# cdglissov/recurrent-flows-msc

Measured on AMD Instinct MI355X. Metric: frames/sec, RFN SM-MNIST 64x64 train step (fwd+bwd+Adam), higher is better.
Workload: dtype f32 (forward convolutions fp32-grade: fused scaled-fp16 split f16x3s / three-piece bf16x6 split; gradient convolutions bf16x3 split MFMA; fp32 accumulate everywhere); 1 GPU; RFN SM-MNIST 64x64 canonical (K=10 L=5 Hd=256 h=200 z=56), global_batch=32, seq_len=20, train step; global_batch=32, seq_len=20, parallelism=dp1

## Files before the change

include/rfn_hip.h:

```cpp
#ifndef RFN_HIP_H
#define RFN_HIP_H

#ifdef __cplusplus
extern "C" {
#endif

typedef void* rfn_stream_t;

int rfn_abi_version(void);
const char* rfn_last_error(void);

int rfn_squeeze2d_f32(const float* x, long x_ns, float* y, long y_ns, int N, int C, int H, int W, int undo,
                      rfn_stream_t stream);

int rfn_channel_stats_f32(const float* x, long x_ns, float* mean, float* var_unbiased, int N, int C, int HW,
                          rfn_stream_t stream);

int rfn_actnorm_invconv_fwd_f32(const float* x, long x_ns, const float* bias, const float* logs, const float* Wm,
                                float* z, long z_ns, int N, int C, int HW, rfn_stream_t stream);
int rfn_actnorm_invconv_bwd_f32(const float* x, long x_ns, const float* bias, const float* logs, const float* Wm,
                                const float* gz, long gz_ns, float* gx, long gx_ns, float* gW, float* gbias,
                                float* glogs, int N, int C, int HW, rfn_stream_t stream);
#define RFN_INVCONV_MAX_STEPS 32
#define RFN_INVCONV_MAX_CHANNELS 96
// ... 50 lines not shown
typedef struct {
    const float* w1;
    const float* w2;
    const float* w3;
    float* dst;
    int Cin, C;
} rfn_po_pack_desc;
int rfn_coupling_po_supported(int N, int C, int Cc, int Hd, int H, int W);
long rfn_coupling_po_packed_bytes(int Cin, int C);
int rfn_coupling_po_pack(const void* descs_device, int n, rfn_stream_t stream);
int rfn_coupling_po_fwd(const float* z, long z_ns, const float* cond, long cond_ns, const void* wpk, const float* n1b,
                        const float* n1l, const float* n2b, const float* n2l, float* h1, long h1_ns, float* h2,
                        long h2_ns, float* P, long P_ns, float* m1, float* m2, int N, int C, int Cc, int H, int W, int act,
                        rfn_stream_t stream);
long rfn_coupling_po_mask_floats(int N, int H, int W);
int rfn_coupling_po_bwd_supported(int N, int C, int H, int W);
long rfn_coupling_po_bwd_packed_bytes(int C);
int rfn_coupling_po_pack_bwd(const void* descs_device, int n, rfn_stream_t stream);
long rfn_coupling_po_bwd_part_floats(int N, int H, int W);
int rfn_coupling_po_bwd(const float* go, long go_ns, const void* wpk, const float* n1l, const float* n2l,
                        const float* m_h1, const float* m_h2, float* ga2, long ga2_ns, float* ga1, long ga1_ns,
                        float* part, int N, int C, int H, int W, int act, rfn_stream_t stream);
int rfn_coupling_po_bwd_finish(const float* const* part, const float* const* w1, const float* const* gw1,
                               const float* const* n1b, const float* const* w2, const float* const* gw2,
                               const float* const* n2b, float* const* out, int n, int nblk, int K1,
                               rfn_stream_t stream);

int rfn_gather_affine_f32(const float* P, const float* o_in, long o_ns, const float* b3, const float* l3, float* o_out,
                          float* z, long z_ns, const float* scale, const float* scale_shift, float* logdet,
                          int clamp_type, int N, int C, int H, int W, rfn_stream_t stream);
// ... 265 lines not shown
```

recurrent-flows-msc_amd/csrc/coupling_po.hip:

```cpp
#include "conv_common.h"

typedef _Float16 f16x8 __attribute__((ext_vector_type(8)));

#define PO_HD 256
#define PO_TAP_PAIRS 5
#define PO_WAVES 4
#define PO_ROUND_PX (32 * PO_WAVES)

struct POGeom {
    int NG, NP, NS1;
    int quad_frags;
    int c3;
    int total_frags;
};
__host__ __device__ static inline POGeom po_geom(int Cin, int C, bool bwd = false) {
    POGeom g;
    g.NG = (Cin + 7) / 8;
    g.NP = bwd ? 0 : (9 * C + 31) / 32;
    g.NS1 = PO_TAP_PAIRS * g.NG;
    g.quad_frags = g.NG * 40 + 4 * 32;
    g.c3 = 1 + 2 * g.quad_frags;
    g.total_frags = g.c3 + 4 * 8 * g.NP;
    return g;
}

__host__ __device__ constexpr int po_gs1(int NG) { return NG > 5 ? 3 : 5; }
__host__ __device__ constexpr int po_gs3(int NP) { return NP > 3 ? 2 : 4; }
__host__ __device__ constexpr int po_group_base(int NG, int NP, int idx) {
    const int QF = NG * 40 + 128, GS1 = po_gs1(NG), NG1 = 5 * NG / GS1, F1 = 8 * GS1;
    return idx < NG1 ? 1 + idx * F1
         : idx < NG1 + 4 ? 1 + NG * 40 + (idx - NG1) * 32
         : idx < 2 * NG1 + 4 ? 1 + QF + (idx - NG1 - 4) * F1
         : idx < 2 * NG1 + 8 ? 1 + QF + NG * 40 + (idx - 2 * NG1 - 4) * 32
         : 1 + 2 * QF + (idx - 2 * NG1 - 8) * 2 * NP * po_gs3(NP);
}
__host__ __device__ constexpr int po_image_positions(int W) {
    return W * W >= PO_ROUND_PX ? (PO_ROUND_PX / W + 2) * (W + 2) : (PO_ROUND_PX / (W * W)) * (W + 2) * (W + 2);
}
__host__ __device__ constexpr int po_slot_frags(int NG, int NP) {
    const int f1 = 8 * po_gs1(NG), f3 = 2 * NP * po_gs3(NP);
    return (f1 > 32 ? f1 : 32) > f3 ? (f1 > 32 ? f1 : 32) : f3;
}
__host__ __device__ constexpr int po_group_size(int NG, int NP, int idx) {
    const int GS1 = po_gs1(NG), NG1 = 5 * NG / GS1, F1 = 8 * GS1;
    return idx < NG1 ? F1 : idx < NG1 + 4 ? 32 : idx < 2 * NG1 + 4 ? F1 : idx < 2 * NG1 + 8 ? 32 : 2 * NP * po_gs3(NP);
}

using POPackDesc = rfn_po_pack_desc;
static_assert(sizeof(rfn_po_pack_desc) == 40, "rfn_po_pack_desc layout is part of the ABI");

__host__ __device__ static inline void po_scale_for_max(float m, float* sc, float* inv) {
    unsigned bits;
    memcpy(&bits, &m, 4);
    int E = (int)((bits >> 23) & 0xff);
    if (E < 40) E = 40;
    if (E > 250) E = 250;
    const unsigned sb = (unsigned)(268 - E) << 23, ib = (unsigned)(E - 14) << 23;
    memcpy(sc, &sb, 4);
    memcpy(inv, &ib, 4);
}
// ... 40 lines not shown
#pragma unroll
    for (int c = 0; c < 3; ++c) scw[c] = 1.0f / d.dst[c];
    const int n1 = 8 * g.NS1, n2 = 8 * 16, n3 = g.NP * 16;
    const long n_items = (long)(n1 + n2 + n3) * 64;
    for (long it = (long)blockIdx.x * blockDim.x + threadIdx.x; it < n_items; it += (long)gridDim.x * blockDim.x) {
        const int lane = (int)(it & 63);
        int k = (int)(it >> 6);
        const int r = lane & 31, kk = lane >> 5;
        float v[8];
#pragma unroll
        for (int j = 0; j < 8; ++j) v[j] = 0.f;
        long frag0;
        float sc;
        if (k < n1) {
            const int a = k / g.NS1, s = k % g.NS1;
            frag0 = 1 + (long)(a >> 2) * g.quad_frags + (s / 5) * 40 + ((s % 5) * 4 + (a & 3)) * 2;
            sc = scw[0];
            const int tp = s / g.NG, gg = s % g.NG, tap = 2 * tp + kk;
            if (tap < 9) {
#pragma unroll
                for (int j = 0; j < 8; ++j) {
                    const int ci = 8 * gg + j;
                    if (ci < Cin)
                        v[j] = BWD ? d.w3[((long)ci * PO_HD + (32 * a + r)) * 9 + (8 - tap)]
                                   : d.w1[((long)(32 * a + r) * Cin + ci) * 9 + tap];
                }
            }
        } else if (k < n1 + n2) {
            k -= n1;
            const int a2 = k >> 4, s = k & 15;
            frag0 = 1 + (long)(s >> 3) * g.quad_frags + g.NG * 40 + ((s & 7) >> 1) * 32 + ((s & 1) * 8 + a2) * 2;
            sc = scw[1];
#pragma unroll
            for (int j = 0; j < 8; ++j) {
                const int c1 = 16 * s + 8 * (j >> 2) + 4 * kk + (j & 3);
                v[j] = BWD ? d.w2[(long)c1 * PO_HD + (32 * a2 + r)] : d.w2[(long)(32 * a2 + r) * PO_HD + c1];
            }
        } else {
            k -= n1 + n2;
            const int jt = k >> 4, s = k & 15;
            frag0 = g.c3 + (long)(s >> 2) * (8 * g.NP) + ((s & 3) * g.NP + jt) * 2;
            sc = scw[2];
            const int R = 32 * jt + r;
            if (R < 9 * d.C) {
                const int tap = R / d.C, co = R % d.C;
#pragma unroll
                for (int j = 0; j < 8; ++j) {
                    const int c2 = 16 * s + 8 * (j >> 2) + 4 * kk + (j & 3);
                    v[j] = d.w3[((long)co * PO_HD + c2) * 9 + tap];
                }
            }
        }
        f16x8 hi, lo;
        po_split_f16(v, sc, hi, lo);
        dst[frag0 * 64 + lane] = hi;
        dst[(frag0 + 1) * 64 + lane] = lo;
    }
}

extern "C" long rfn_coupling_po_packed_bytes(int Cin, int C) { return (long)po_geom(Cin, C).total_frags * 1024; }
extern "C" long rfn_coupling_po_bwd_packed_bytes(int C) { return (long)po_geom(C, C, true).total_frags * 1024; }

extern "C" int rfn_coupling_po_pack(const void* descs_device, int n, rfn_stream_t stream) {
    RFN_CHECK_ARG(descs_device && n >= 0, -1);
    if (n == 0) return 0;
    hipLaunchKernelGGL(po_pack_scale_kernel<false>, dim3(3, n), dim3(256), 0, (hipStream_t)stream,
                       reinterpret_cast<const POPackDesc*>(descs_device));
    hipLaunchKernelGGL(po_pack_fwd_kernel<false>, dim3(16, n), dim3(256), 0, (hipStream_t)stream,
                       reinterpret_cast<const POPackDesc*>(descs_device));
    RFN_LAUNCH_CHECK();
    return 0;
}

extern "C" int rfn_coupling_po_pack_bwd(const void* descs_device, int n, rfn_stream_t stream) {
    RFN_CHECK_ARG(descs_device && n >= 0, -1);
    if (n == 0) return 0;
// ... 68 lines not shown
        float s01 = (bit0 ? t4[1] : t4[0]) +
                    __int_as_float(__builtin_amdgcn_update_dpp(0, __float_as_int(bit0 ? t4[0] : t4[1]), 0xB1, 0xF, 0xF, true));
        float s23 = (bit0 ? t4[3] : t4[2]) +
                    __int_as_float(__builtin_amdgcn_update_dpp(0, __float_as_int(bit0 ? t4[2] : t4[3]), 0xB1, 0xF, 0xF, true));
        psum[q] += (bit1 ? s23 : s01) +
                   __int_as_float(__builtin_amdgcn_update_dpp(0, __float_as_int(bit1 ? s01 : s23), 0x4E, 0xF, 0xF, true));
    }
}

__device__ __forceinline__ int po_exp_of(const float m) {
    int E = (int)((__float_as_uint(m) >> 23) & 0xff);
    E = E < 40 ? 40 : E;
    return E > 250 ? 250 : E;
}

template <int NG, int NP, int LOGW, int ACT, bool BWD>
__global__ __launch_bounds__(64 * PO_WAVES) void coupling_po_fwd_kernel(const POFwdParams p) {
    constexpr int W = 1 << LOGW, HW = W * W, IW = W + 2;
    constexpr int FPR = HW >= PO_ROUND_PX ? 1 : PO_ROUND_PX / HW;
    constexpr int RROWS = HW >= PO_ROUND_PX ? PO_ROUND_PX / W : W;
    constexpr int FPOS = (RROWS + 2) * IW, IPOS = FPR * FPOS;
    constexpr int PO_ITEMS = (NG * IPOS + 64 * PO_WAVES - 1) / (64 * PO_WAVES);
    constexpr int RPF_SHIFT = HW >= PO_ROUND_PX ? 2 * LOGW - 7 : 0;
    constexpr int GS1 = po_gs1(NG), NG1 = 5 * NG / GS1;
    constexpr int GS3 = po_gs3(NP), NG3 = 16 / GS3;
    constexpr bool RT = NG > 5;
    constexpr bool LATE = RT || (BWD && NG > 1);
    constexpr bool NOHOIST = LATE || NG == 5;
    static_assert((5 * NG) % GS1 == 0 && (!RT || NG % GS1 == 0), "conv1 grouping");
    constexpr int G3 = 2 * NP * GS3;
    constexpr int Y1 = 2 * GS1, Y3 = G3 / 4;
    static_assert(G3 % 4 == 0, "a group's fragments are shared evenly by the four waves");
    constexpr int SLOTF = po_slot_frags(NG, NP);
    constexpr int SLOT = SLOTF * 1024;
    extern __shared__ __attribute__((aligned(16))) unsigned char lds[];
    constexpr int NGRP = 2 * NG1 + 8 + (BWD ? 0 : NG3);
    float* par = reinterpret_cast<float*>(lds + 3 * SLOT);
    float* red = par + 1024;
    f16x8* img = reinterpret_cast<f16x8*>(lds + 3 * SLOT + 4096 + 64);
    float* gsum = reinterpret_cast<float*>(lds + 3 * SLOT + 4096 + 64 + 2 * NG * IPOS * 16);
    const int tid = threadIdx.x, lane = tid & 63;
    const int wave = __builtin_amdgcn_readfirstlane(tid >> 6);
    const int l31 = lane & 31, kk = lane >> 5;
    const int Cin = p.Ch + p.Cc;
    constexpr unsigned ch_bytes = (unsigned)HW * 4u;

    for (int c = tid; c < 256; c += 64 * PO_WAVES) {
        par[c] = BWD ? 0.f : p.n1b[c];
        par[256 + c] = expf(p.n1l[c]);
        par[512 + c] = BWD ? 0.f : p.n2b[c];
        par[768 + c] = expf(p.n2l[c]);
    }
    float ps1[BWD ? 8 : 1][4], ps2[BWD ? 8 : 1][4];
#pragma unroll
    for (int a = 0; a < (BWD ? 8 : 1); ++a)
#pragma unroll
        for (int q = 0; q < 4; ++q) ps1[a][q] = ps2[a][q] = 0.f;
    const bool lbit0 = lane & 1, lbit1 = lane & 2;
    const float* hdr = reinterpret_cast<const float*>(p.wpk);
// ... 3 lines not shown
    int sl = 2;
    auto dma = [&](const int base, const int nfr, const int slot) {
        const unsigned char* src = p.wpk + (long)(base + wave) * 1024 + lane * 16;
        unsigned char* dst = lds + slot * SLOT + wave * 1024;
        for (int i = wave; i < nfr; i += PO_WAVES, src += PO_WAVES * 1024, dst += PO_WAVES * 1024)
            __builtin_amdgcn_global_load_lds((const __attribute__((address_space(1))) void*)src,
                                             (__attribute__((address_space(3))) void*)dst, 16, 0, 0);
    };
#define PO_BOUNDARY(IDX, YOUNGER)                                                                          \
    do {                                                                                                   \
        po_wait_vm<(YOUNGER) < 63 ? (YOUNGER) : 63>();                                                     \
        __builtin_amdgcn_s_barrier();                                                                      \
        const int free_slot = sl;                                                                          \
        sl = sl == 2 ? 0 : sl + 1;                                                                         \
        const int n2_ = (IDX) + 2;                                                                         \
        if (n2_ < NGRP) dma(po_group_base(NG, NP, n2_), po_group_size(NG, NP, n2_), free_slot);            \
        else if (more) dma(po_group_base(NG, NP, n2_ - NGRP), po_group_size(NG, NP, n2_ - NGRP), free_slot); \
    } while (0)

    const auto rs_h1 = __builtin_amdgcn_make_buffer_rsrc(p.h1, 0, 0xFFFFFFFFu, 0x00020000);
    const auto rs_h2 = __builtin_amdgcn_make_buffer_rsrc(p.h2, 0, 0xFFFFFFFFu, 0x00020000);

    float raw[PO_ITEMS][8];
    auto stage_load = [&](const int rnd) {
        const int n0_ = FPR > 1 ? rnd * FPR : rnd >> RPF_SHIFT;
        const int y0_ = FPR > 1 ? 0 : ((rnd & ((1 << RPF_SHIFT) - 1)) * PO_ROUND_PX) >> LOGW;
        int tid_ = tid;
        if (NOHOIST) asm volatile("" : "+v"(tid_));
#pragma unroll
        for (int it = 0; it < PO_ITEMS; ++it) {
            const int item = tid_ + it * 64 * PO_WAVES;
            const bool live = item < NG * IPOS;
            const int g = live ? item / IPOS : 0, pos = live ? item - g * IPOS : 0;
            const int fr = FPR > 1 ? pos / FPOS : 0, rem = pos - fr * FPOS;
            const int iy = rem / IW, ix = rem - iy * IW;
            const int gy = y0_ - 1 + iy, gx = ix - 1;
            const bool ok = live && gy >= 0 && gy < W && gx >= 0 && gx < W;
            const int off = ok ? gy * W + gx : 0;
            const float* zb = p.z + (long)(n0_ + fr) * p.z_ns;
            const float* cb = p.cond + (long)(n0_ + fr) * p.cond_ns;
#pragma unroll
            for (int j = 0; j < 8; ++j) {
                const int ci = 8 * g + j;
                const int cc = ci < Cin ? ci : 0;
                const float* src = cc < p.Ch ? zb + (long)cc * HW : cb + (long)(cc - p.Ch) * HW;
                raw[it][j] = src[off];
            }
        }
    };
    float u1_next = 0.f;
    auto stage_finish = [&](const int rnd) {
        const int y0_ = FPR > 1 ? 0 : ((rnd & ((1 << RPF_SHIFT) - 1)) * PO_ROUND_PX) >> LOGW;
        float vm = 0.f;
        int tid_ = tid;
        if (NOHOIST) asm volatile("" : "+v"(tid_));
#pragma unroll
        for (int it = 0; it < PO_ITEMS; ++it) {
            const int item = tid_ + it * 64 * PO_WAVES;
            const bool live = item < NG * IPOS;
            const int g = live ? item / IPOS : 0, pos = live ? item - g * IPOS : 0;
            const int rem = FPR > 1 ? pos % FPOS : pos;
            const int iy = rem / IW, ix = rem - iy * IW;
            const int gy = y0_ - 1 + iy, gx = ix - 1;
            const bool ok = live && gy >= 0 && gy < W && gx >= 0 && gx < W;
#pragma unroll
            for (int j = 0; j < 8; ++j) {
                raw[it][j] = (ok && 8 * g + j < Cin) ? raw[it][j] : 0.f;
                vm = fmaxf(vm, fabsf(raw[it][j]));
            }
        }
#pragma unroll
        for (int off = 32; off > 0; off >>= 1) vm = fmaxf(vm, __shfl_xor(vm, off, 64));
        if (lane == 0) red[wave] = vm;
        asm volatile("s_waitcnt lgkmcnt(0)" ::: "memory");
        __builtin_amdgcn_s_barrier();
        vm = fmaxf(fmaxf(red[0], red[1]), fmaxf(red[2], red[3]));
        const int Eimg = po_exp_of(vm);
        const float sc_img = __uint_as_float((unsigned)(268 - Eimg) << 23);
        u1_next = __uint_as_float((unsigned)(Eimg - 14) << 23) * inv_w1;
#pragma unroll
        for (int it = 0; it < PO_ITEMS; ++it) {
            const int item = tid_ + it * 64 * PO_WAVES;
            if (item < NG * IPOS) {
                const int g = item / IPOS, pos = item - g * IPOS;
                f16x8 hi, lo;
                po_split_f16(raw[it], sc_img, hi, lo);
                img[(0 * NG + g) * IPOS + pos] = hi;
                img[(1 * NG + g) * IPOS + pos] = lo;
            }
        }
        asm volatile("s_waitcnt lgkmcnt(0)" ::: "memory");
    };

    int round = blockIdx.x;
    if (round < p.n_rounds) {
        const bool more = true;
        (void)more;
        dma(po_group_base(NG, NP, 0), po_group_size(NG, NP, 0), 0);
        dma(po_group_base(NG, NP, 1), po_group_size(NG, NP, 1), 1);
        stage_load(round);
        stage_finish(round);
    }
    for (; round < p.n_rounds; round += gridDim.x) {
        const bool more = round + (int)gridDim.x < p.n_rounds;
        const int rp = 32 * wave + l31;
        const int fr = FPR > 1 ? rp >> (2 * LOGW) : 0;
        const int n = FPR > 1 ? round * FPR + fr : round >> RPF_SHIFT;
        const int pix = FPR > 1 ? rp & (HW - 1) : (round & ((1 << RPF_SHIFT) - 1)) * PO_ROUND_PX + rp;
        const int y0 = FPR > 1 ? 0 : ((round & ((1 << RPF_SHIFT) - 1)) * PO_ROUND_PX) >> LOGW;
        const float u1 = u1_next;

        const int iy = (pix >> LOGW) - y0 + 1, ix = (pix & (W - 1)) + 1;
        const f16x8* bp[PO_TAP_PAIRS];
#pragma unroll
        for (int tp = 0; tp < PO_TAP_PAIRS; ++tp) {
            const int tA = 2 * tp, tB = 2 * tp + 1 < 9 ? 2 * tp + 1 : 4;
            const int dy = kk ? (tB / 3 - 1) : (tA / 3 - 1);
            const int dx = kk ? (tB % 3 - 1) : (tA % 3 - 1);
            bp[tp] = img + fr * FPOS + (iy + dy) * IW + ix + dx;
        }
        const unsigned vo1 = (unsigned)(((long)n * p.h1_ns + (long)(4 * kk) * HW + pix) * 4);
        const unsigned vo2 = (unsigned)(((long)n * p.h2_ns + (long)(4 * kk) * HW + pix) * 4);
        const float* par1 = par + 4 * kk;
        const float* par2 = par + 512 + 4 * kk;

        unsigned mk1[4] = {0u, 0u, 0u, 0u}, mk2[4] = {0u, 0u, 0u, 0u};
        if (BWD && ACT != 0) {
            const uint4 a_ = reinterpret_cast<const uint4*>(p.m1)[(long)round * (64 * PO_WAVES) + tid];
            const uint4 b_ = reinterpret_cast<const uint4*>(p.m2)[(long)round * (64 * PO_WAVES) + tid];
            mk1[0] = a_.x; mk1[1] = a_.y; mk1[2] = a_.z; mk1[3] = a_.w;
            mk2[0] = b_.x; mk2[1] = b_.y; mk2[2] = b_.z; mk2[3] = b_.w;
        }

        f32x16 acc2[8];
#pragma unroll
// ... 16 lines not shown
                _Pragma("unroll") for (int t = 0; t < 4; ++t) PO_MFMA(Q[t], A[cur][t][1], B[cur][0]);      \
                __builtin_amdgcn_sched_barrier(0);                                                         \
                if (!(LAST)) {                                                                             \
                    _Pragma("unroll") for (int t = 0; t < 4; ++t) {                                        \
                        A[nxt][t][0] = fr[((ANEXT) * 4 + t) * 2 * 64];                                     \
                        A[nxt][t][1] = fr[(((ANEXT) * 4 + t) * 2 + 1) * 64];                               \
                    }                                                                                      \
                    _Pragma("unroll") for (int pl = 0; pl < 2; ++pl) B[nxt][pl] = BNEXT;                   \
                }                                                                                          \
                __builtin_amdgcn_sched_barrier(0);                                                         \
                _Pragma("unroll") for (int t = 0; t < 4; ++t) PO_MFMA(Q[t], A[cur][t][0], B[cur][1]);      \
                _Pragma("unroll") for (int t = 0; t < 4; ++t) PO_MFMA(Q[t], A[cur][t][0], B[cur][0]);      \
                __builtin_amdgcn_sched_barrier(0);                                                         \
            } while (0)
            if constexpr (!RT) {
#pragma unroll
            for (int gi = 0; gi < NG1; ++gi) {
                if (u == 1 && gi < 2 && more && !LATE) {
                    if (gi + 1 < NG1) PO_BOUNDARY(u * (NG1 + 4) + gi, Y1 + 8 * PO_ITEMS);
                    else PO_BOUNDARY(u * (NG1 + 4) + gi, 8 + 8 * PO_ITEMS);
                } else {
                    if (gi + 1 < NG1) PO_BOUNDARY(u * (NG1 + 4) + gi, Y1);
                    else PO_BOUNDARY(u * (NG1 + 4) + gi, 8);
                }
                const f16x8* fr = reinterpret_cast<const f16x8*>(lds + sl * SLOT) + lane;
                f16x8 A[2][4][2], B[2][2];
#pragma unroll
                for (int t = 0; t < 4; ++t) {
                    A[0][t][0] = fr[(t * 2) * 64];
                    A[0][t][1] = fr[(t * 2 + 1) * 64];
                }
#pragma unroll
                for (int pl = 0; pl < 2; ++pl) B[0][pl] = bp[(GS1 * gi) / NG][(pl * NG + (GS1 * gi) % NG) * IPOS];
#pragma unroll
                for (int k = 0; k < GS1; ++k) {
                    const int s = GS1 * gi + k, cur = k & 1, nxt = cur ^ 1;
                    PO_C1_STEP(k + 1 == GS1, k + 1, bp[(s + 1) / NG][(pl * NG + (s + 1) % NG) * IPOS]);
                }
            }
            } else {
#pragma unroll
            for (int tp = 0; tp < PO_TAP_PAIRS; ++tp) {
#pragma unroll 1
                for (int gg = 0; gg < NG / GS1; ++gg) {
                    const int gq = tp * (NG / GS1) + gg;
                    const int gidx = u * (NG1 + 4) + gq;
                    if (u == 1 && tp == 0 && gg < 2 && more && !LATE) PO_BOUNDARY(gidx, Y1 + 8 * PO_ITEMS);
                    else PO_BOUNDARY(gidx, Y1);
                    const f16x8* fr = reinterpret_cast<const f16x8*>(lds + sl * SLOT) + lane;
                    const f16x8* bq = bp[tp] + (GS1 * gg) * IPOS;
                    f16x8 A[2][4][2], B[2][2];
#pragma unroll
                    for (int t = 0; t < 4; ++t) {
                        A[0][t][0] = fr[(t * 2) * 64];
                        A[0][t][1] = fr[(t * 2 + 1) * 64];
                    }
#pragma unroll
                    for (int pl = 0; pl < 2; ++pl) B[0][pl] = bq[(pl * NG) * IPOS];
#pragma unroll
                    for (int k = 0; k < GS1; ++k) {
                        const int cur = k & 1, nxt = cur ^ 1;
                        PO_C1_STEP(k + 1 == GS1, k + 1, bq[(pl * NG + k + 1) * IPOS]);
                    }
                }
            }
            }
#undef PO_C1_STEP
            float vmax = 0.f;
            unsigned mq[2] = {0u, 0u};
#pragma unroll
            for (int t = 0; t < 4; ++t) {
                const int a = 4 * u + t;
                if (BWD)
                    po_epilogue_bwd<ACT>(Q[t], u1, par1 + 256 + 32 * a, rs_h1, vo1 + (unsigned)(32 * a) * ch_bytes, ch_bytes,
                                         vmax, mk1[a >> 1] >> (16 * (a & 1)), ps1[BWD ? a : 0], lbit0, lbit1);
                else if (t & 1)
                    po_epilogue<ACT, 16>(Q[t], u1, par1 + 32 * a, rs_h1, vo1 + (unsigned)(32 * a) * ch_bytes, ch_bytes,
                                         vmax, mq[t >> 1]);
                else
// ... 170 lines not shown
            for (int a = 0; a < 8; ++a)
#pragma unroll
                for (int q = 0; q < 4; ++q) {
                    float v = st == 0 ? ps1[a][q] : ps2[a][q];
                    v += __int_as_float(__builtin_amdgcn_update_dpp(0, __float_as_int(v), 0x124, 0xF, 0xF, true));
                    v += __int_as_float(__builtin_amdgcn_update_dpp(0, __float_as_int(v), 0x128, 0xF, 0xF, true));
                    v += __shfl_xor(v, 16, 64);
                    if (l31 < 4) gsum[(wave * 2 + st) * 256 + 32 * a + 4 * kk + 8 * q + l31] = v;
                }
        __syncthreads();
        for (int c = tid; c < 512; c += 64 * PO_WAVES)
            p.part[(long)blockIdx.x * 512 + c] = (gsum[c] + gsum[512 + c]) + (gsum[1024 + c] + gsum[1536 + c]);
    }
}

template <int NG, int NP, int LOGW, int ACT, bool BWD>
static int launch_po_fwd_t(const POFwdParams& p, hipStream_t s) {
    constexpr int SLOTF = po_slot_frags(NG, NP);
    constexpr int W = 1 << LOGW, IPOS = po_image_positions(W);
    const size_t ldsz = (size_t)3 * SLOTF * 1024 + 4096 + 64 + (size_t)2 * NG * IPOS * 16 + (BWD ? PO_WAVES * 512 * 4 : 0);
    if (ldsz > 160 * 1024 || IPOS != p.IPOS) {
        rfn_set_error("coupling_po: %zu bytes of LDS / %d image positions (expected %d)", ldsz, p.IPOS, IPOS);
        return -5;
    }
    auto kern = coupling_po_fwd_kernel<NG, NP, LOGW, ACT, BWD>;
    (void)hipFuncSetAttribute((const void*)kern, hipFuncAttributeMaxDynamicSharedMemorySize, (int)ldsz);
    const int grid = p.n_rounds < 256 ? p.n_rounds : 256;
    hipLaunchKernelGGL(kern, dim3(grid), dim3(64 * PO_WAVES), ldsz, s, p);
    return 0;
}

template <int NG, int NP, int LOGW, bool BWD = false>
static int launch_po_fwd(const POFwdParams& p, hipStream_t s) {
    if (p.act == 1) return launch_po_fwd_t<NG, NP, LOGW, 1, BWD>(p, s);
    if (p.act == 2) return launch_po_fwd_t<NG, NP, LOGW, 2, BWD>(p, s);
    return launch_po_fwd_t<NG, NP, LOGW, 0, BWD>(p, s);
}

static bool po_fwd_instance(int NG, int NP, int W) {
    return (NG == 3 && NP == 2 && W == 32) || (NG == 5 && NP == 3 && W == 16) || (NG == 9 && NP == 5 && W == 8) ||
           (NG == 9 && NP == 4 && W == 32);
}
extern "C" int rfn_coupling_po_supported(int N, int C, int Cc, int Hd, int H, int W) {
    if (N <= 0 || C <= 0 || C % 2 || Cc < 0 || H <= 0 || W <= 0) return 0;
    const POGeom g = po_geom(C / 2 + Cc, C);
    const bool pow2 = (H & (H - 1)) == 0 && (W & (W - 1)) == 0;
    const bool inst = H == W && po_fwd_instance(g.NG, g.NP, W);
    const bool small = (long)N * PO_HD * H * W * 4 < (1L << 32);
    return Hd == PO_HD && pow2 && W <= PO_ROUND_PX && ((long)N * H * W) % PO_ROUND_PX == 0 && inst && small;
}

// ... 18 lines not shown
    RFN_CHECK_ARG(z && wpk && n1b && n1l && n2b && n2l && h1 && h2 && P && (Cc == 0 || cond), -1);
    RFN_CHECK_ARG(rfn_coupling_po_supported(N, C, Cc, PO_HD, H, W), -2);
    RFN_CHECK_ARG(((uintptr_t)wpk & 15) == 0 && ((uintptr_t)m1 & 15) == 0 && ((uintptr_t)m2 & 15) == 0, -3);
    RFN_CHECK_ARG(h1_ns * 4L * N < (1L << 32) && h2_ns * 4L * N < (1L << 32), -4);
    POFwdParams p;
    memset(&p, 0, sizeof(p));
    p.z = z; p.z_ns = z_ns; p.cond = cond ? cond : z; p.cond_ns = cond_ns;
    p.wpk = reinterpret_cast<const unsigned char*>(wpk);
    p.n1b = n1b; p.n1l = n1l; p.n2b = n2b; p.n2l = n2l;
    p.h1 = h1; p.h1_ns = h1_ns; p.h2 = h2; p.h2_ns = h2_ns; p.P = P; p.P_ns = P_ns;
    p.m1 = reinterpret_cast<unsigned*>(m1); p.m2 = reinterpret_cast<unsigned*>(m2);
    p.Ch = C / 2; p.Cc = Cc;
    po_fill_geometry(p, N, C, H, W, act);
    const POGeom g = po_geom(p.Ch + Cc, C);
    int rc = -4;
    if (g.NG == 3 && g.NP == 2 && W == 32) rc = launch_po_fwd<3, 2, 5>(p, (hipStream_t)stream);
    if (g.NG == 5 && g.NP == 3 && W == 16) rc = launch_po_fwd<5, 3, 4>(p, (hipStream_t)stream);
    if (g.NG == 9 && g.NP == 5 && W == 8) rc = launch_po_fwd<9, 5, 3>(p, (hipStream_t)stream);
    if (g.NG == 9 && g.NP == 4 && W == 32) rc = launch_po_fwd<9, 4, 5>(p, (hipStream_t)stream);
    if (rc) return rc;
    RFN_LAUNCH_CHECK();
    return 0;
}

static bool po_bwd_instance(int NG, int W) {
    return (NG == 1 && (W == 32 || W == 16)) || (NG == 2 && (W == 8 || W == 32));
}
extern "C" int rfn_coupling_po_bwd_supported(int N, int C, int H, int W) {
    if (N <= 0 || C <= 0 || H != W) return 0;
    const bool small = (long)N * PO_HD * H * W * 4 < (1L << 32);
    return po_bwd_instance((C + 7) / 8, W) && ((long)N * H * W) % PO_ROUND_PX == 0 && small;
}
// ... 5 lines not shown
    RFN_CHECK_ARG(((uintptr_t)wpk & 15) == 0 && ((uintptr_t)m_h1 & 15) == 0 && ((uintptr_t)m_h2 & 15) == 0, -3);
    RFN_CHECK_ARG(ga1_ns * 4L * N < (1L << 32) && ga2_ns * 4L * N < (1L << 32), -4);
    POFwdParams p;
    memset(&p, 0, sizeof(p));
    p.z = go; p.z_ns = go_ns; p.cond = go; p.cond_ns = 0;
    p.wpk = reinterpret_cast<const unsigned char*>(wpk);
    p.n1b = n2l; p.n1l = n2l; p.n2b = n1l; p.n2l = n1l;
    p.h1 = ga2; p.h1_ns = ga2_ns; p.h2 = ga1; p.h2_ns = ga1_ns;
    p.m1 = reinterpret_cast<unsigned*>(const_cast<float*>(m_h2));
    p.m2 = reinterpret_cast<unsigned*>(const_cast<float*>(m_h1));
    p.part = part;
    p.Ch = C; p.Cc = 0;
    po_fill_geometry(p, N, C, H, W, act);
    int rc = -4;
    const int NGb = (C + 7) / 8;
    if (NGb == 1 && W == 32) rc = launch_po_fwd<1, 0, 5, true>(p, (hipStream_t)stream);
    if (NGb == 1 && W == 16) rc = launch_po_fwd<1, 0, 4, true>(p, (hipStream_t)stream);
    if (NGb == 2 && W == 8) rc = launch_po_fwd<2, 0, 3, true>(p, (hipStream_t)stream);
    if (NGb == 2 && W == 32) rc = launch_po_fwd<2, 0, 5, true>(p, (hipStream_t)stream);
    if (rc) return rc;
    RFN_LAUNCH_CHECK();
    return 0;
}

#define PO_FIN_MAX 16
struct POFinishParams {
    const float* part[PO_FIN_MAX];
    const float* w1[PO_FIN_MAX]; const float* gw1[PO_FIN_MAX]; const float* n1b[PO_FIN_MAX];
    const float* w2[PO_FIN_MAX]; const float* gw2[PO_FIN_MAX]; const float* n2b[PO_FIN_MAX];
    float* out[PO_FIN_MAX];
    int nblk, K1;
};
// ... 50 lines not shown
```

Before: 11920 frames/s.

## Pack partial channel groups across taps to skip zero-padded conv1 K-steps

Replaces the fixed tap-pair K ordering of the first coupling convolution with a per-instance unit order. When the input channel count leaves a small remainder modulo 8, the leftover channels of several taps are packed into one 8-wide fragment instead of being zero-padded per tap, which reduces the number of MFMA K-steps and packed weight fragments. The weight packer, ring-group DMA bases and sizes, LDS sizing and B-operand loads are all re-derived from this order, and new template instances are used for the narrow shapes. The cost is more complex address generation (sub-16-byte LDS gathers for the leftover units) and more kernel instantiations.

```diff
diff --git a/include/rfn_hip.h b/include/rfn_hip.h
--- a/include/rfn_hip.h
+++ b/include/rfn_hip.h
@@ -88,6 +88,10 @@
                         long h2_ns, float* P, long P_ns, float* m1, float* m2, int N, int C, int Cc, int H, int W, int act,
                         rfn_stream_t stream);
 long rfn_coupling_po_mask_floats(int N, int H, int W);
+int rfn_coupling_po_k_order(int Cin, int bwd, int unit, long long* tap0, long long* n_taps, long long* ch0,
+                            long long* n_ch);
+int rfn_coupling_po_ring_group(int Cin, int C, int bwd, int idx, long long* first_frag, long long* n_frags);
+long rfn_coupling_po_lds_bytes(int Cin, int C, int W, int bwd);
 int rfn_coupling_po_bwd_supported(int N, int C, int H, int W);
 long rfn_coupling_po_bwd_packed_bytes(int C);
 int rfn_coupling_po_pack_bwd(const void* descs_device, int n, rfn_stream_t stream);
diff --git a/recurrent-flows-msc_amd/csrc/coupling_po.hip b/recurrent-flows-msc_amd/csrc/coupling_po.hip
--- a/recurrent-flows-msc_amd/csrc/coupling_po.hip
+++ b/recurrent-flows-msc_amd/csrc/coupling_po.hip
@@ -1,11 +1,62 @@
 #include "conv_common.h"
 
 typedef _Float16 f16x8 __attribute__((ext_vector_type(8)));
+typedef unsigned u32x4 __attribute__((ext_vector_type(4)));
 
 #define PO_HD 256
-#define PO_TAP_PAIRS 5
 #define PO_WAVES 4
 #define PO_ROUND_PX (32 * PO_WAVES)
+
+struct POOrder {
+    int NG, NGT, RP, R;
+    int n_units, NS1;
+};
+struct POUnit {
+    int tap0, n_taps, ch0, n_ch;
+    int w;
+    int g;
+};
+__host__ __device__ constexpr bool po_narrow(int NG, int rp, bool bwd) {
+    return bwd ? (NG == 1 && rp == 4) : ((NG == 3 && rp == 2) || (NG == 5 && rp == 4));
+}
+__host__ __device__ constexpr POOrder po_order(int Cin, bool bwd) {
+    POOrder o{};
+    o.NG = (Cin + 7) / 8;
+    o.R = Cin % 8;
+    const int rp = o.R == 0 ? 0 : o.R <= 2 ? 2 : o.R <= 4 ? 4 : 8;
+    o.RP = po_narrow(o.NG, rp, bwd) ? rp : 0;
+    o.NGT = o.RP ? o.NG - 1 : o.NG;
+    o.n_units = 9 * o.NGT + (o.RP ? (9 * o.RP + 7) / 8 : 0);
+    o.NS1 = (o.n_units + 1) / 2;
+    return o;
+}
+__host__ __device__ constexpr int po_tap_off(int tap, int IW) { return (tap / 3 - 1) * IW + (tap % 3 - 1); }
+__host__ __device__ constexpr int po_group_ch0(const POOrder& o, int g) { return o.RP ? (g < o.NGT ? o.R + 8 * g : 0) : 8 * g; }
+__host__ __device__ constexpr int po_group_nch(const POOrder& o, int Cin, int g) {
+    const int n = o.RP && g == o.NGT ? o.R : Cin - po_group_ch0(o, g);
+    return n < 8 ? n : 8;
+}
+__host__ __device__ constexpr POUnit po_unit(int Cin, bool bwd, int u) {
+    const POOrder o = po_order(Cin, bwd);
+    POUnit q{};
+    q.w = 8;
+    if (u < 0 || u >= o.n_units) {
+        q.tap0 = 4;
+        return q;
+    }
+    if (u < 9 * o.NGT) {
+        q.tap0 = u / o.NGT; q.n_taps = 1; q.g = u % o.NGT;
+        q.ch0 = po_group_ch0(o, q.g);
+        q.n_ch = po_group_nch(o, Cin, q.g);
+        return q;
+    }
+    const int tpu = 8 / o.RP;
+    q.w = o.RP; q.g = o.NGT;
+    q.tap0 = (u - 9 * o.NGT) * tpu;
+    q.n_taps = 9 - q.tap0 < tpu ? 9 - q.tap0 : tpu;
+    q.ch0 = po_group_ch0(o, q.g); q.n_ch = po_group_nch(o, Cin, q.g);
+    return q;
+}
 
 struct POGeom {
     int NG, NP, NS1;
@@ -13,12 +64,12 @@
     int c3;
     int total_frags;
 };
-__host__ __device__ static inline POGeom po_geom(int Cin, int C, bool bwd = false) {
-    POGeom g;
+__host__ __device__ constexpr POGeom po_geom(int Cin, int C, bool bwd = false) {
+    POGeom g{};
     g.NG = (Cin + 7) / 8;
     g.NP = bwd ? 0 : (9 * C + 31) / 32;
-    g.NS1 = PO_TAP_PAIRS * g.NG;
-    g.quad_frags = g.NG * 40 + 4 * 32;
+    g.NS1 = po_order(Cin, bwd).NS1;
+    g.quad_frags = g.NS1 * 8 + 4 * 32;
     g.c3 = 1 + 2 * g.quad_frags;
     g.total_frags = g.c3 + 4 * 8 * g.NP;
     return g;
@@ -26,24 +77,38 @@
 
 __host__ __device__ constexpr int po_gs1(int NG) { return NG > 5 ? 3 : 5; }
 __host__ __device__ constexpr int po_gs3(int NP) { return NP > 3 ? 2 : 4; }
-__host__ __device__ constexpr int po_group_base(int NG, int NP, int idx) {
-    const int QF = NG * 40 + 128, GS1 = po_gs1(NG), NG1 = 5 * NG / GS1, F1 = 8 * GS1;
-    return idx < NG1 ? 1 + idx * F1
-         : idx < NG1 + 4 ? 1 + NG * 40 + (idx - NG1) * 32
-         : idx < 2 * NG1 + 4 ? 1 + QF + (idx - NG1 - 4) * F1
-         : idx < 2 * NG1 + 8 ? 1 + QF + NG * 40 + (idx - 2 * NG1 - 4) * 32
+__host__ __device__ constexpr int po_ng1(int NG, int NS1) { return (NS1 + po_gs1(NG) - 1) / po_gs1(NG); }
+__host__ __device__ constexpr int po_g1_first(int NG, int NS1, int gi) {
+    const int n = po_ng1(NG, NS1), rem = NS1 % n;
+    return gi * (NS1 / n) + (gi < rem ? gi : rem);
+}
+__host__ __device__ constexpr int po_g1_steps(int NG, int NS1, int gi) {
+    const int n = po_ng1(NG, NS1);
+    return NS1 / n + (gi < NS1 % n ? 1 : 0);
+}
+__host__ __device__ constexpr int po_group_base(int NG, int NS1, int NP, int idx) {
+    const int QF = NS1 * 8 + 128, NG1 = po_ng1(NG, NS1);
+    return idx < NG1 ? 1 + 8 * po_g1_first(NG, NS1, idx)
+         : idx < NG1 + 4 ? 1 + NS1 * 8 + (idx - NG1) * 32
+         : idx < 2 * NG1 + 4 ? 1 + QF + 8 * po_g1_first(NG, NS1, idx - NG1 - 4)
+         : idx < 2 * NG1 + 8 ? 1 + QF + NS1 * 8 + (idx - 2 * NG1 - 4) * 32
          : 1 + 2 * QF + (idx - 2 * NG1 - 8) * 2 * NP * po_gs3(NP);
 }
 __host__ __device__ constexpr int po_image_positions(int W) {
     return W * W >= PO_ROUND_PX ? (PO_ROUND_PX / W + 2) * (W + 2) : (PO_ROUND_PX / (W * W)) * (W + 2) * (W + 2);
 }
-__host__ __device__ constexpr int po_slot_frags(int NG, int NP) {
-    const int f1 = 8 * po_gs1(NG), f3 = 2 * NP * po_gs3(NP);
+__host__ __device__ constexpr int po_slot_frags(int NG, int NS1, int NP) {
+    const int f1 = 8 * po_g1_steps(NG, NS1, 0), f3 = 2 * NP * po_gs3(NP);
     return (f1 > 32 ? f1 : 32) > f3 ? (f1 > 32 ? f1 : 32) : f3;
 }
-__host__ __device__ constexpr int po_group_size(int NG, int NP, int idx) {
-    const int GS1 = po_gs1(NG), NG1 = 5 * NG / GS1, F1 = 8 * GS1;
-    return idx < NG1 ? F1 : idx < NG1 + 4 ? 32 : idx < 2 * NG1 + 4 ? F1 : idx < 2 * NG1 + 8 ? 32 : 2 * NP * po_gs3(NP);
+__host__ __device__ constexpr int po_group_size(int NG, int NS1, int NP, int idx) {
+    const int NG1 = po_ng1(NG, NS1);
+    return idx < NG1 ? 8 * po_g1_steps(NG, NS1, idx) : idx < NG1 + 4 ? 32
+         : idx < 2 * NG1 + 4 ? 8 * po_g1_steps(NG, NS1, idx - NG1 - 4) : idx < 2 * NG1 + 8 ? 32 : 2 * NP * po_gs3(NP);
+}
+__host__ __device__ constexpr long po_lds_bytes(int NG, int NS1, int NP, int W, bool bwd) {
+    return 3L * po_slot_frags(NG, NS1, NP) * 1024 + 4096 + 64 + 2L * NG * po_image_positions(W) * 16 +
+           (bwd ? PO_WAVES * 512 * 4 : 0);
 }
 
 using POPackDesc = rfn_po_pack_desc;
@@ -114,22 +179,20 @@
         float sc;
         if (k < n1) {
             const int a = k / g.NS1, s = k % g.NS1;
-            frag0 = 1 + (long)(a >> 2) * g.quad_frags + (s / 5) * 40 + ((s % 5) * 4 + (a & 3)) * 2;
+            frag0 = 1 + (long)(a >> 2) * g.quad_frags + (s * 4 + (a & 3)) * 2;
             sc = scw[0];
-            const int tp = s / g.NG, gg = s % g.NG, tap = 2 * tp + kk;
-            if (tap < 9) {
-#pragma unroll
-                for (int j = 0; j < 8; ++j) {
-                    const int ci = 8 * gg + j;
-                    if (ci < Cin)
-                        v[j] = BWD ? d.w3[((long)ci * PO_HD + (32 * a + r)) * 9 + (8 - tap)]
-                                   : d.w1[((long)(32 * a + r) * Cin + ci) * 9 + tap];
-                }
+            const POUnit q = po_unit(Cin, BWD, 2 * s + kk);
+#pragma unroll
+            for (int j = 0; j < 8; ++j) {
+                const int t = j / q.w, c = j % q.w, tap = q.tap0 + t, ci = q.ch0 + c;
+                if (t < q.n_taps && c < q.n_ch)
+                    v[j] = BWD ? d.w3[((long)ci * PO_HD + (32 * a + r)) * 9 + (8 - tap)]
+                               : d.w1[((long)(32 * a + r) * Cin + ci) * 9 + tap];
             }
         } else if (k < n1 + n2) {
             k -= n1;
             const int a2 = k >> 4, s = k & 15;
-            frag0 = 1 + (long)(s >> 3) * g.quad_frags + g.NG * 40 + ((s & 7) >> 1) * 32 + ((s & 1) * 8 + a2) * 2;
+            frag0 = 1 + (long)(s >> 3) * g.quad_frags + g.NS1 * 8 + ((s & 7) >> 1) * 32 + ((s & 1) * 8 + a2) * 2;
             sc = scw[1];
 #pragma unroll
             for (int j = 0; j < 8; ++j) {
@@ -160,6 +223,32 @@
 
 extern "C" long rfn_coupling_po_packed_bytes(int Cin, int C) { return (long)po_geom(Cin, C).total_frags * 1024; }
 extern "C" long rfn_coupling_po_bwd_packed_bytes(int C) { return (long)po_geom(C, C, true).total_frags * 1024; }
+
+extern "C" int rfn_coupling_po_k_order(int Cin, int bwd, int unit, long long* tap0, long long* n_taps, long long* ch0,
+                                       long long* n_ch) {
+    RFN_CHECK_ARG(Cin > 0, -1);
+    const POOrder o = po_order(Cin, bwd != 0);
+    if (unit < 0) return o.n_units;
+    RFN_CHECK_ARG(unit < o.n_units && tap0 && n_taps && ch0 && n_ch, -2);
+    const POUnit q = po_unit(Cin, bwd != 0, unit);
+    *tap0 = q.tap0; *n_taps = q.n_taps; *ch0 = q.ch0; *n_ch = q.n_ch;
+    return unit / 2;
+}
+extern "C" int rfn_coupling_po_ring_group(int Cin, int C, int bwd, int idx, long long* first_frag, long long* n_frags) {
+    RFN_CHECK_ARG(Cin > 0 && (bwd || C > 0), -1);
+    const POGeom g = po_geom(Cin, C, bwd != 0);
+    const int n = 2 * po_ng1(g.NG, g.NS1) + 8 + (bwd ? 0 : 16 / po_gs3(g.NP));
+    if (idx < 0) return n;
+    RFN_CHECK_ARG(idx < n && first_frag && n_frags, -2);
+    *first_frag = po_group_base(g.NG, g.NS1, g.NP, idx);
+    *n_frags = po_group_size(g.NG, g.NS1, g.NP, idx);
+    return 0;
+}
+extern "C" long rfn_coupling_po_lds_bytes(int Cin, int C, int W, int bwd) {
+    RFN_CHECK_ARG(Cin > 0 && W > 0 && (bwd || C > 0), -1);
+    const POGeom g = po_geom(Cin, C, bwd != 0);
+    return po_lds_bytes(g.NG, g.NS1, g.NP, W, bwd != 0);
+}
 
 extern "C" int rfn_coupling_po_pack(const void* descs_device, int n, rfn_stream_t stream) {
     RFN_CHECK_ARG(descs_device && n >= 0, -1);
@@ -258,24 +347,30 @@
     return E > 250 ? 250 : E;
 }
 
-template <int NG, int NP, int LOGW, int ACT, bool BWD>
+template <int NG, int NP, int LOGW, int ACT, bool BWD, int RP>
 __global__ __launch_bounds__(64 * PO_WAVES) void coupling_po_fwd_kernel(const POFwdParams p) {
+    constexpr int CREP = RP ? 8 * (NG - 1) + RP : 8 * NG;
+    constexpr POOrder ORD = po_order(CREP, BWD);
+    static_assert(ORD.NG == NG && ORD.RP == RP, "instantiation outside po_order");
+    static_assert(RP == 0 || (9 * ORD.NGT) % 2 == 0, "a k-step is two full or two leftover units");
+    constexpr int NS1 = ORD.NS1;
     constexpr int W = 1 << LOGW, HW = W * W, IW = W + 2;
     constexpr int FPR = HW >= PO_ROUND_PX ? 1 : PO_ROUND_PX / HW;
     constexpr int RROWS = HW >= PO_ROUND_PX ? PO_ROUND_PX / W : W;
     constexpr int FPOS = (RROWS + 2) * IW, IPOS = FPR * FPOS;
     constexpr int PO_ITEMS = (NG * IPOS + 64 * PO_WAVES - 1) / (64 * PO_WAVES);
     constexpr int RPF_SHIFT = HW >= PO_ROUND_PX ? 2 * LOGW - 7 : 0;
-    constexpr int GS1 = po_gs1(NG), NG1 = 5 * NG / GS1;
+    constexpr int GS1 = po_gs1(NG), NG1 = po_ng1(NG, NS1);
     constexpr int GS3 = po_gs3(NP), NG3 = 16 / GS3;
     constexpr bool RT = NG > 5;
     constexpr bool LATE = RT || (BWD && NG > 1);
     constexpr bool NOHOIST = LATE || NG == 5;
-    static_assert((5 * NG) % GS1 == 0 && (!RT || NG % GS1 == 0), "conv1 grouping");
+    static_assert(!RT || (RP == 0 && NG % GS1 == 0 && NG1 == 4 * (NG / GS1) + (NG / 2 + GS1) / GS1 &&
+                          po_g1_steps(NG, NS1, NG1 - 2) == GS1), "conv1 grouping");
     constexpr int G3 = 2 * NP * GS3;
-    constexpr int Y1 = 2 * GS1, Y3 = G3 / 4;
+    constexpr int Y1 = 2 * po_g1_steps(NG, NS1, 0), Y3 = G3 / 4;
     static_assert(G3 % 4 == 0, "a group's fragments are shared evenly by the four waves");
-    constexpr int SLOTF = po_slot_frags(NG, NP);
+    constexpr int SLOTF = po_slot_frags(NG, NS1, NP);
     constexpr int SLOT = SLOTF * 1024;
     extern __shared__ __attribute__((aligned(16))) unsigned char lds[];
     constexpr int NGRP = 2 * NG1 + 8 + (BWD ? 0 : NG3);
@@ -287,6 +382,7 @@
     const int wave = __builtin_amdgcn_readfirstlane(tid >> 6);
     const int l31 = lane & 31, kk = lane >> 5;
     const int Cin = p.Ch + p.Cc;
+    const POOrder ordr = po_order(Cin, BWD);
     constexpr unsigned ch_bytes = (unsigned)HW * 4u;
 
     for (int c = tid; c < 256; c += 64 * PO_WAVES) {
@@ -320,8 +416,8 @@
         const int free_slot = sl;                                                                          \
         sl = sl == 2 ? 0 : sl + 1;                                                                         \
         const int n2_ = (IDX) + 2;                                                                         \
-        if (n2_ < NGRP) dma(po_group_base(NG, NP, n2_), po_group_size(NG, NP, n2_), free_slot);            \
-        else if (more) dma(po_group_base(NG, NP, n2_ - NGRP), po_group_size(NG, NP, n2_ - NGRP), free_slot); \
+        if (n2_ < NGRP) dma(po_group_base(NG, NS1, NP, n2_), po_group_size(NG, NS1, NP, n2_), free_slot);            \
+        else if (more) dma(po_group_base(NG, NS1, NP, n2_ - NGRP), po_group_size(NG, NS1, NP, n2_ - NGRP), free_slot); \
     } while (0)
 
     const auto rs_h1 = __builtin_amdgcn_make_buffer_rsrc(p.h1, 0, 0xFFFFFFFFu, 0x00020000);
@@ -345,10 +441,10 @@
             const int off = ok ? gy * W + gx : 0;
             const float* zb = p.z + (long)(n0_ + fr) * p.z_ns;
             const float* cb = p.cond + (long)(n0_ + fr) * p.cond_ns;
+            const int c0 = po_group_ch0(ordr, g), nc = po_group_nch(ordr, Cin, g);
 #pragma unroll
             for (int j = 0; j < 8; ++j) {
-                const int ci = 8 * g + j;
-                const int cc = ci < Cin ? ci : 0;
+                const int cc = j < nc ? c0 + j : 0;
                 const float* src = cc < p.Ch ? zb + (long)cc * HW : cb + (long)(cc - p.Ch) * HW;
                 raw[it][j] = src[off];
             }
@@ -369,9 +465,10 @@
             const int iy = rem / IW, ix = rem - iy * IW;
             const int gy = y0_ - 1 + iy, gx = ix - 1;
             const bool ok = live && gy >= 0 && gy < W && gx >= 0 && gx < W;
+            const int nc = po_group_nch(ordr, Cin, g);
 #pragma unroll
             for (int j = 0; j < 8; ++j) {
-                raw[it][j] = (ok && 8 * g + j < Cin) ? raw[it][j] : 0.f;
+                raw[it][j] = (ok && j < nc) ? raw[it][j] : 0.f;
                 vm = fmaxf(vm, fabsf(raw[it][j]));
             }
         }
@@ -402,8 +499,8 @@
     if (round < p.n_rounds) {
         const bool more = true;
         (void)more;
-        dma(po_group_base(NG, NP, 0), po_group_size(NG, NP, 0), 0);
-        dma(po_group_base(NG, NP, 1), po_group_size(NG, NP, 1), 1);
+        dma(po_group_base(NG, NS1, NP, 0), po_group_size(NG, NS1, NP, 0), 0);
+        dma(po_group_base(NG, NS1, NP, 1), po_group_size(NG, NS1, NP, 1), 1);
         stage_load(round);
         stage_finish(round);
     }
@@ -417,14 +514,32 @@
         const float u1 = u1_next;
 
         const int iy = (pix >> LOGW) - y0 + 1, ix = (pix & (W - 1)) + 1;
-        const f16x8* bp[PO_TAP_PAIRS];
-#pragma unroll
-        for (int tp = 0; tp < PO_TAP_PAIRS; ++tp) {
-            const int tA = 2 * tp, tB = 2 * tp + 1 < 9 ? 2 * tp + 1 : 4;
-            const int dy = kk ? (tB / 3 - 1) : (tA / 3 - 1);
-            const int dx = kk ? (tB % 3 - 1) : (tA % 3 - 1);
-            bp[tp] = img + fr * FPOS + (iy + dy) * IW + ix + dx;
-        }
+        const f16x8* pc = img + fr * FPOS + iy * IW + ix;
+        auto load_b = [&](const int s, const int pl) __attribute__((always_inline)) -> f16x8 {
+            const POUnit qa = po_unit(CREP, BWD, 2 * s), qb = po_unit(CREP, BWD, 2 * s + 1);
+            int kk = lane >> 5;
+            asm volatile("" : "+v"(kk));
+            if (RP == 0 || 2 * s < 9 * ORD.NGT) {
+                const int oa = po_tap_off(qa.tap0, IW) + (pl * NG + qa.g) * IPOS;
+                const int ob = po_tap_off(qb.tap0, IW) + (pl * NG + qb.g) * IPOS;
+                return pc[oa + kk * (ob - oa)];
+            }
+            constexpr int WB = RP ? RP : 8, T = 8 / WB;
+            const unsigned char* base = reinterpret_cast<const unsigned char*>(pc + (pl * NG + NG - 1) * IPOS);
+            u32x4 d;
+#pragma unroll
+            for (int t = 0; t < T; ++t) {
+                const int oa = 16 * po_tap_off(t < qa.n_taps ? qa.tap0 + t : 4, IW);
+                const int ob = 16 * po_tap_off(t < qb.n_taps ? qb.tap0 + t : 4, IW);
+                if (WB == 4) {
+                    const uint2 v = *reinterpret_cast<const uint2*>(base + (kk ? ob : oa));
+                    d[(2 * t) & 3] = v.x; d[(2 * t + 1) & 3] = v.y;
+                } else {
+                    d[t & 3] = *reinterpret_cast<const unsigned*>(base + (kk ? ob : oa));
+                }
+            }
+            return __builtin_bit_cast(f16x8, d);
+        };
         const unsigned vo1 = (unsigned)(((long)n * p.h1_ns + (long)(4 * kk) * HW + pix) * 4);
         const unsigned vo2 = (unsigned)(((long)n * p.h2_ns + (long)(4 * kk) * HW + pix) * 4);
         const float* par1 = par + 4 * kk;
@@ -471,14 +586,19 @@
                 __builtin_amdgcn_sched_barrier(0);                                                         \
             } while (0)
             if constexpr (!RT) {
+            constexpr int KA = po_g1_steps(NG, NS1, 0), KB = po_g1_steps(NG, NS1, NG1 - 1);
 #pragma unroll
             for (int gi = 0; gi < NG1; ++gi) {
+                const int s0 = po_g1_first(NG, NS1, gi), KN = po_g1_steps(NG, NS1, gi);
+                const bool lastg = gi + 1 == NG1, nextA = !lastg && po_g1_steps(NG, NS1, gi + 1) == KA;
                 if (u == 1 && gi < 2 && more && !LATE) {
-                    if (gi + 1 < NG1) PO_BOUNDARY(u * (NG1 + 4) + gi, Y1 + 8 * PO_ITEMS);
-                    else PO_BOUNDARY(u * (NG1 + 4) + gi, 8 + 8 * PO_ITEMS);
+                    if (lastg) PO_BOUNDARY(u * (NG1 + 4) + gi, 8 + 8 * PO_ITEMS);
+                    else if (nextA) PO_BOUNDARY(u * (NG1 + 4) + gi, 2 * KA + 8 * PO_ITEMS);
+                    else PO_BOUNDARY(u * (NG1 + 4) + gi, 2 * KB + 8 * PO_ITEMS);
                 } else {
-                    if (gi + 1 < NG1) PO_BOUNDARY(u * (NG1 + 4) + gi, Y1);
-                    else PO_BOUNDARY(u * (NG1 + 4) + gi, 8);
+                    if (lastg) PO_BOUNDARY(u * (NG1 + 4) + gi, 8);
+                    else if (nextA) PO_BOUNDARY(u * (NG1 + 4) + gi, 2 * KA);
+                    else PO_BOUNDARY(u * (NG1 + 4) + gi, 2 * KB);
                 }
                 const f16x8* fr = reinterpret_cast<const f16x8*>(lds + sl * SLOT) + lane;
                 f16x8 A[2][4][2], B[2][2];
@@ -488,38 +608,51 @@
                     A[0][t][1] = fr[(t * 2 + 1) * 64];
                 }
 #pragma unroll
-                for (int pl = 0; pl < 2; ++pl) B[0][pl] = bp[(GS1 * gi) / NG][(pl * NG + (GS1 * gi) % NG) * IPOS];
+                for (int pl = 0; pl < 2; ++pl) B[0][pl] = load_b(s0, pl);
 #pragma unroll
                 for (int k = 0; k < GS1; ++k) {
-                    const int s = GS1 * gi + k, cur = k & 1, nxt = cur ^ 1;
-                    PO_C1_STEP(k + 1 == GS1, k + 1, bp[(s + 1) / NG][(pl * NG + (s + 1) % NG) * IPOS]);
+                    if (k < KN) {
+                        const int s = s0 + k, cur = k & 1, nxt = cur ^ 1;
+                        PO_C1_STEP(k + 1 == KN, k + 1, load_b(s + 1, pl));
+                    }
                 }
             }
             } else {
-#pragma unroll
-            for (int tp = 0; tp < PO_TAP_PAIRS; ++tp) {
+            auto c1_group = [&](const int tp, const int gg, const int KN) __attribute__((always_inline)) {
+                const int gidx = u * (NG1 + 4) + tp * (NG / GS1) + gg;
+                if (tp < 4) PO_BOUNDARY(gidx, 2 * GS1);
+                else if (KN == GS1) PO_BOUNDARY(gidx, 2 * po_g1_steps(NG, NS1, NG1 - 1));
+                else PO_BOUNDARY(gidx, 8);
+                const f16x8* fr = reinterpret_cast<const f16x8*>(lds + sl * SLOT) + lane;
+                const f16x8* pa = pc + po_tap_off(2 * tp, IW);
+                const int dsel = (tp < 4 ? po_tap_off(2 * tp + 1, IW) - po_tap_off(2 * tp, IW) : 0) - NG * IPOS;
+                const int u0 = 2 * GS1 * gg + kk;
+                auto b_at = [&](const int k, const int pl) __attribute__((always_inline)) -> f16x8 {
+                    const int uu = u0 + 2 * k;
+                    return pa[(pl * NG + uu) * IPOS + (uu >= NG ? dsel : 0)];
+                };
+                f16x8 A[2][4][2], B[2][2];
+#pragma unroll
+                for (int t = 0; t < 4; ++t) {
+                    A[0][t][0] = fr[(t * 2) * 64];
+                    A[0][t][1] = fr[(t * 2 + 1) * 64];
+                }
+#pragma unroll
+                for (int pl = 0; pl < 2; ++pl) B[0][pl] = b_at(0, pl);
+#pragma unroll
+                for (int k = 0; k < GS1; ++k) {
+                    if (k < KN) {
+                        const int cur = k & 1, nxt = cur ^ 1;
+                        PO_C1_STEP(k + 1 == KN, k + 1, b_at(k + 1, pl));
+                    }
+                }
+            };
+#pragma unroll
+            for (int tp = 0; tp < 5; ++tp) {
+                const int nfull = tp < 4 ? NG / GS1 : (NG + 1) / 2 / GS1;
 #pragma unroll 1
-                for (int gg = 0; gg < NG / GS1; ++gg) {
-                    const int gq = tp * (NG / GS1) + gg;
-                    const int gidx = u * (NG1 + 4) + gq;
-                    if (u == 1 && tp == 0 && gg < 2 && more && !LATE) PO_BOUNDARY(gidx, Y1 + 8 * PO_ITEMS);
-                    else PO_BOUNDARY(gidx, Y1);
-                    const f16x8* fr = reinterpret_cast<const f16x8*>(lds + sl * SLOT) + lane;
-                    const f16x8* bq = bp[tp] + (GS1 * gg) * IPOS;
-                    f16x8 A[2][4][2], B[2][2];
-#pragma unroll
-                    for (int t = 0; t < 4; ++t) {
-                        A[0][t][0] = fr[(t * 2) * 64];
-                        A[0][t][1] = fr[(t * 2 + 1) * 64];
-                    }
-#pragma unroll
-                    for (int pl = 0; pl < 2; ++pl) B[0][pl] = bq[(pl * NG) * IPOS];
-#pragma unroll
-                    for (int k = 0; k < GS1; ++k) {
-                        const int cur = k & 1, nxt = cur ^ 1;
-                        PO_C1_STEP(k + 1 == GS1, k + 1, bq[(pl * NG + k + 1) * IPOS]);
-                    }
-                }
+                for (int gg = 0; gg < nfull; ++gg) c1_group(tp, gg, GS1);
+                if (tp == 4 && (NG + 1) / 2 % GS1) c1_group(tp, nfull, (NG + 1) / 2 % GS1);
             }
             }
 #undef PO_C1_STEP
@@ -720,27 +853,34 @@
     }
 }
 
-template <int NG, int NP, int LOGW, int ACT, bool BWD>
+template <int NG, int NP, int LOGW, int ACT, bool BWD, int RP>
 static int launch_po_fwd_t(const POFwdParams& p, hipStream_t s) {
-    constexpr int SLOTF = po_slot_frags(NG, NP);
     constexpr int W = 1 << LOGW, IPOS = po_image_positions(W);
-    const size_t ldsz = (size_t)3 * SLOTF * 1024 + 4096 + 64 + (size_t)2 * NG * IPOS * 16 + (BWD ? PO_WAVES * 512 * 4 : 0);
+    constexpr int NS1 = po_order(RP ? 8 * (NG - 1) + RP : 8 * NG, BWD).NS1;
+    constexpr size_t ldsz = (size_t)po_lds_bytes(NG, NS1, NP, W, BWD);
     if (ldsz > 160 * 1024 || IPOS != p.IPOS) {
         rfn_set_error("coupling_po: %zu bytes of LDS / %d image positions (expected %d)", ldsz, p.IPOS, IPOS);
         return -5;
     }
-    auto kern = coupling_po_fwd_kernel<NG, NP, LOGW, ACT, BWD>;
+    auto kern = coupling_po_fwd_kernel<NG, NP, LOGW, ACT, BWD, RP>;
     (void)hipFuncSetAttribute((const void*)kern, hipFuncAttributeMaxDynamicSharedMemorySize, (int)ldsz);
     const int grid = p.n_rounds < 256 ? p.n_rounds : 256;
     hipLaunchKernelGGL(kern, dim3(grid), dim3(64 * PO_WAVES), ldsz, s, p);
     return 0;
 }
 
-template <int NG, int NP, int LOGW, bool BWD = false>
+template <int NG, int NP, int LOGW, bool BWD, int RP>
+static int launch_po_fwd_r(const POFwdParams& p, hipStream_t s) {
+    if (p.act == 1) return launch_po_fwd_t<NG, NP, LOGW, 1, BWD, RP>(p, s);
+    if (p.act == 2) return launch_po_fwd_t<NG, NP, LOGW, 2, BWD, RP>(p, s);
+    return launch_po_fwd_t<NG, NP, LOGW, 0, BWD, RP>(p, s);
+}
+template <int NG, int NP, int LOGW, bool BWD = false, int NRP = 0>
 static int launch_po_fwd(const POFwdParams& p, hipStream_t s) {
-    if (p.act == 1) return launch_po_fwd_t<NG, NP, LOGW, 1, BWD>(p, s);
-    if (p.act == 2) return launch_po_fwd_t<NG, NP, LOGW, 2, BWD>(p, s);
-    return launch_po_fwd_t<NG, NP, LOGW, 0, BWD>(p, s);
+    static_assert(NRP == 0 || po_narrow(NG, NRP, BWD), "narrow instantiation outside po_narrow");
+    if (NRP != 0 && po_order(p.Ch + p.Cc, BWD).RP == NRP) return launch_po_fwd_r<NG, NP, LOGW, BWD, NRP>(p, s);
+    if (po_order(p.Ch + p.Cc, BWD).RP != 0) return -4;
+    return launch_po_fwd_r<NG, NP, LOGW, BWD, 0>(p, s);
 }
 
 static bool po_fwd_instance(int NG, int NP, int W) {
@@ -789,8 +929,8 @@
     po_fill_geometry(p, N, C, H, W, act);
     const POGeom g = po_geom(p.Ch + Cc, C);
     int rc = -4;
-    if (g.NG == 3 && g.NP == 2 && W == 32) rc = launch_po_fwd<3, 2, 5>(p, (hipStream_t)stream);
-    if (g.NG == 5 && g.NP == 3 && W == 16) rc = launch_po_fwd<5, 3, 4>(p, (hipStream_t)stream);
+    if (g.NG == 3 && g.NP == 2 && W == 32) rc = launch_po_fwd<3, 2, 5, false, 2>(p, (hipStream_t)stream);
+    if (g.NG == 5 && g.NP == 3 && W == 16) rc = launch_po_fwd<5, 3, 4, false, 4>(p, (hipStream_t)stream);
     if (g.NG == 9 && g.NP == 5 && W == 8) rc = launch_po_fwd<9, 5, 3>(p, (hipStream_t)stream);
     if (g.NG == 9 && g.NP == 4 && W == 32) rc = launch_po_fwd<9, 4, 5>(p, (hipStream_t)stream);
     if (rc) return rc;
@@ -826,8 +966,8 @@
     po_fill_geometry(p, N, C, H, W, act);
     int rc = -4;
     const int NGb = (C + 7) / 8;
-    if (NGb == 1 && W == 32) rc = launch_po_fwd<1, 0, 5, true>(p, (hipStream_t)stream);
-    if (NGb == 1 && W == 16) rc = launch_po_fwd<1, 0, 4, true>(p, (hipStream_t)stream);
+    if (NGb == 1 && W == 32) rc = launch_po_fwd<1, 0, 5, true, 4>(p, (hipStream_t)stream);
+    if (NGb == 1 && W == 16) rc = launch_po_fwd<1, 0, 4, true, 4>(p, (hipStream_t)stream);
     if (NGb == 2 && W == 8) rc = launch_po_fwd<2, 0, 3, true>(p, (hipStream_t)stream);
     if (NGb == 2 && W == 32) rc = launch_po_fwd<2, 0, 5, true>(p, (hipStream_t)stream);
     if (rc) return rc;
```

After: 12050 frames/s (median of 6 runs). +1.1%, better.
